# glennhickey/teHmm

Hardware: AMD Instinct MI355X
Metric: genome positions/sec (Viterbi+posterior), 35 states x 10 tracks (higher is better)
Workload: dtype f64

## Files before the change

### include/tehmm_hip.h

```cpp
#ifndef TEHMM_HIP_H
#define TEHMM_HIP_H

#include <stdint.h>

#ifdef __cplusplus
extern "C" {
#endif

#define TEHMM_OK 0
#define TEHMM_ERR_ARG (-1)
#define TEHMM_ERR_HIP (-2)
#define TEHMM_ERR_UNSUPPORTED (-3)

int tehmm_abi_version(void);
const char *tehmm_last_error(void);
int tehmm_device_count(int *count);
int tehmm_set_device(int device);
int tehmm_max_states(void);
int tehmm_max_states_any(void);


int tehmm_emission_u8(int64_t T, int K, int N, int S, const uint8_t *obs, const double *logProbs,
                      double normalize, const double *segRatios, double *outProbs);
int tehmm_emission_u16(int64_t T, int K, int N, int S, const uint16_t *obs, const double *logProbs,
// ... 19 lines not shown
                            const double *posteriors, const double *segRatios);
int tehmm_accumulate_obs_u16(int64_t T, int K, int N, int S, const uint16_t *obs, double *obsStats,
                             const double *posteriors, const double *segRatios);
int tehmm_accumulate_obs_i32(int64_t T, int K, int N, int S, const int32_t *obs, double *obsStats,
                             const double *posteriors, const double *segRatios);

int tehmm_update_counts_u8(int64_t T, int K, int N, int S, const uint8_t *obs, int n_intervals,
                           const int64_t *starts, const int64_t *ends, const int32_t *states,
                           const double *segRatios, double *obsStats);
int tehmm_update_counts_u16(int64_t T, int K, int N, int S, const uint16_t *obs, int n_intervals,
                            const int64_t *starts, const int64_t *ends, const int32_t *states,
                            const double *segRatios, double *obsStats);
int tehmm_update_counts_i32(int64_t T, int K, int N, int S, const int32_t *obs, int n_intervals,
                            const int64_t *starts, const int64_t *ends, const int32_t *states,
                            const double *segRatios, double *obsStats);

typedef struct tehmm_model tehmm_model_t;
typedef struct tehmm_batch tehmm_batch_t;

int tehmm_model_create(int N, int K, int S, const double *log_transmat, const double *log_startprob,
                       const double *logProbs, double normalize, const int32_t *symbolsPerTrack,
                       tehmm_model_t **out);
int tehmm_model_destroy(tehmm_model_t *model);

int tehmm_batch_create(int n_intervals, const int64_t *offsets, int K, const uint8_t *obs,
                       const double *segRatios, int obs_on_device, tehmm_batch_t **out);
int tehmm_batch_create_u16(int n_intervals, const int64_t *offsets, int K, const uint16_t *obs,
                           const double *segRatios, tehmm_batch_t **out);
int tehmm_batch_create_i32(int n_intervals, const int64_t *offsets, int K, const int32_t *obs,
                           const double *segRatios, tehmm_batch_t **out);
int tehmm_batch_destroy(tehmm_batch_t *batch);
int64_t tehmm_batch_total(const tehmm_batch_t *batch);
int tehmm_batch_reset_cache(tehmm_batch_t *batch);

#define TEHMM_EVAL_VITERBI 1
#define TEHMM_EVAL_POSTERIOR 2
#define TEHMM_EVAL_USE_RATIOS 4

int tehmm_eval_batch(tehmm_model_t *model, tehmm_batch_t *batch, int flags,
                     double *viterbi_logprob, double *forward_logprob);

int tehmm_batch_get_paths(tehmm_batch_t *batch, int64_t row0, int64_t row1, int64_t *paths);
int tehmm_batch_get_posteriors(tehmm_batch_t *batch, int64_t row0, int64_t row1, double *post);
int tehmm_host_alloc(size_t bytes, void **out);
int tehmm_host_free(void *ptr);
int tehmm_trim_pools(void);
// ... 44 lines not shown
```

### tehmm_amd/_lib.py

```python
import ctypes
import os

import numpy as np

_HERE = os.path.dirname(os.path.abspath(__file__))
LIB_PATH = os.environ.get("TEHMM_HIP_LIB") or os.path.join(_HERE, "libtehmm_hip.so")

f64p = ctypes.POINTER(ctypes.c_double)
i64p = ctypes.POINTER(ctypes.c_int64)
i32p = ctypes.POINTER(ctypes.c_int32)
u8p = ctypes.POINTER(ctypes.c_uint8)
vp = ctypes.c_void_p
c_i64 = ctypes.c_int64
c_int = ctypes.c_int
c_dbl = ctypes.c_double

SIGNATURES = {
    "tehmm_abi_version": (c_int, []),
    "tehmm_last_error": (ctypes.c_char_p, []),
    "tehmm_device_count": (c_int, [ctypes.POINTER(c_int)]),
    "tehmm_set_device": (c_int, [c_int]),
    "tehmm_max_states": (c_int, []),
    "tehmm_max_states_any": (c_int, []),
    "tehmm_emission_u8": (c_int, [c_i64, c_int, c_int, c_int, vp, f64p, c_dbl, f64p, f64p]),
# ... 21 lines not shown
    "tehmm_model_get_params": (c_int, [vp, f64p, f64p, f64p]),
    "tehmm_segment_table_u8": (c_int, [c_i64, c_int, u8p, c_i64, i64p, u8p, f64p, u8p, f64p]),
    "tehmm_mask_table_u8": (c_int, [c_i64, c_int, u8p, c_int, u8p, u8p, i32p, u8p, i32p, i64p]),
    "tehmm_batch_get_interval_logprobs": (c_int, [vp, f64p]),
    "tehmm_batch_posterior_masksum": (c_int, [vp, f64p, c_i64, c_i64, f64p]),
    "tehmm_bed_coords": (c_int, [c_i64, c_i64, c_i64, i64p, i32p, c_i64, i64p, i64p]),
    "tehmm_write_bed": (c_int, [ctypes.c_char_p, c_int, ctypes.c_char_p, c_i64, i64p, i64p, i64p, c_int,
                                ctypes.POINTER(ctypes.c_char_p), f64p]),
    "tehmm_model_create": (c_int, [c_int, c_int, c_int, f64p, f64p, f64p, c_dbl, i32p,
                                   ctypes.POINTER(vp)]),
    "tehmm_model_destroy": (c_int, [vp]),
    "tehmm_batch_create": (c_int, [c_int, i64p, c_int, vp, vp, c_int, ctypes.POINTER(vp)]),
    "tehmm_batch_create_u16": (c_int, [c_int, i64p, c_int, vp, vp, ctypes.POINTER(vp)]),
    "tehmm_batch_create_i32": (c_int, [c_int, i64p, c_int, vp, vp, ctypes.POINTER(vp)]),
    "tehmm_batch_destroy": (c_int, [vp]),
    "tehmm_batch_total": (c_i64, [vp]),
    "tehmm_batch_reset_cache": (c_int, [vp]),
    "tehmm_eval_batch": (c_int, [vp, vp, c_int, f64p, f64p]),
    "tehmm_batch_get_paths": (c_int, [vp, c_i64, c_i64, i64p]),
    "tehmm_batch_get_posteriors": (c_int, [vp, c_i64, c_i64, f64p]),
    "tehmm_host_alloc": (c_int, [ctypes.c_size_t, ctypes.POINTER(vp)]),
    "tehmm_host_free": (c_int, [vp]),
    "tehmm_trim_pools": (c_int, []),
    "tehmm_batch_device_ptrs": (c_int, [vp, ctypes.POINTER(vp), ctypes.POINTER(vp)]),
    "tehmm_estep_batch": (c_int, [vp, vp, c_int, f64p, f64p, f64p, f64p]),
    "tehmm_batch_last_timing": (c_int, [vp, c_int, ctypes.POINTER(ctypes.c_char_p), f64p]),
    "tehmm_debug_read_stamps": (c_int, [ctypes.POINTER(ctypes.c_uint64), c_int]),
}

EVAL_VITERBI = 1
EVAL_POSTERIOR = 2
EVAL_USE_RATIOS = 4

_lib = None


class TeHmmHipError(RuntimeError):
    code = 0


def load():
    global _lib
    if _lib is None:
        if not os.path.exists(LIB_PATH):
            raise TeHmmHipError(
                "%s not found: build it with `python -m tehmm_amd.build` (hipcc, gfx950). "
# ... 77 lines not shown
```

### tehmm_amd/csrc/tehmm_aux_host.inc

```

int tehmm_segment_table_u8(int64_t T, int K, const uint8_t *data, int64_t n_seg, const int64_t *segOffsets,
                           const uint8_t *is_gaussian, const double *mapback, uint8_t *out, double *means) {
  if (T <= 0 || K <= 0 || K > TEHMM_MAX_TRACKS || n_seg <= 0 || !data || !segOffsets || !is_gaussian || !out || !means)
    return fail(TEHMM_ERR_ARG, "tehmm_segment_table_u8: bad argument");
  bool any_gauss = false;
  for (int k = 0; k < K; ++k) any_gauss = any_gauss || is_gaussian[k] != 0;
  if (any_gauss && !mapback) return fail(TEHMM_ERR_ARG, "tehmm_segment_table_u8: gaussian track without a map-back table");
  for (int64_t i = 0; i < n_seg; ++i)
    if (segOffsets[i] < 0 || segOffsets[i] >= T || (i > 0 && segOffsets[i] <= segOffsets[i - 1]))
      return fail(TEHMM_ERR_ARG, "tehmm_segment_table_u8: segment offsets must be ascending and inside the table");
  DBuf<uint8_t> d_data, d_g, d_out;
  DBuf<int64_t> d_off;
  DBuf<double> d_mb, d_means;
  HIPCHK(d_data.upload(data, (size_t)T * K));
  HIPCHK(d_off.upload(segOffsets, (size_t)n_seg));
  HIPCHK(d_g.upload(is_gaussian, (size_t)K));
  if (mapback) HIPCHK(d_mb.upload(mapback, (size_t)K * 256));
  HIPCHK(d_out.alloc((size_t)n_seg * K));
  HIPCHK(d_means.alloc((size_t)n_seg * K));
  hipLaunchKernelGGL(k_segment_table, dim3(grid_for(n_seg, 4, 16384)), dim3(256), 0, 0, T, K,
                     (const uint8_t *)d_data.p, n_seg, (const int64_t *)d_off.p, (const uint8_t *)d_g.p,
                     (const double *)d_mb.p, d_out.p, d_means.p);
  HIPCHK(hipGetLastError());
  HIPCHK(hipMemcpy(out, d_out.p, (size_t)n_seg * K, hipMemcpyDeviceToHost));
// ... 95 lines not shown
  const int N = m->N, NP = m->NP;
  const MstepTracks tr = mstep_tracks(m);
  if (update_start || update_trans)
    hipLaunchKernelGGL(k_mstep_trans, dim3(1), dim3(128), 0, 0, N, NP, dev_stats, update_start, update_trans,
                       startprob_prior, transmat_prior, m->lt.p, m->pi.p);
  if (update_emission) {
    hipLaunchKernelGGL(k_mstep_emis, dim3(grid_for((int64_t)m->K * N, 64)), dim3(64), 0, 0, tr, N, NP, dev_stats,
                       fudge, m->tab.p);
    if (n_gauss > 0) {
      DBuf<int> d_gt;
      DBuf<double> d_val, d_gp;
      HIPCHK(d_gt.upload(gauss_tracks, (size_t)n_gauss));
      HIPCHK(d_val.upload(gauss_values, (size_t)n_gauss * m->S));
      HIPCHK(d_gp.alloc((size_t)n_gauss * N * 2));
      hipLaunchKernelGGL(k_mstep_gauss, dim3(grid_for((int64_t)n_gauss * N, 64)), dim3(64), 0, 0, tr, n_gauss,
                         (const int *)d_gt.p, (const double *)d_val.p, m->S, N, NP, uniform_mix, m->tab.p, d_gp.p);
      HIPCHK(hipGetLastError());
      if (gauss_params)
        HIPCHK(hipMemcpy(gauss_params, d_gp.p, (size_t)n_gauss * N * 2 * sizeof(double), hipMemcpyDeviceToHost));
      else
        HIPCHK(hipDeviceSynchronize());
    }
    if (int rcp = build_ptab(m)) return rcp;
    if (m->lds_rows > 0) {
      DBuf<int> d_lb;
      HIPCHK(d_lb.upload(m->ldsbase, (size_t)m->K));
      hipLaunchKernelGGL(k_model_ltab, dim3(m->K), dim3(256), 0, 0, tr, (const int *)d_lb.p, NP,
                         (const double *)m->tab.p, m->ltab.p);
      HIPCHK(hipDeviceSynchronize());
    }
  }
  if (update_trans) {
    hipLaunchKernelGGL(k_model_layouts, dim3(grid_for((int64_t)NP * NP, 256)), dim3(256), 0, 0, NP,
                       (const double *)m->lt.p, m->ltT.p, m->A.p, m->AT.p, m->ltG.p, m->AG.p, m->ATG.p, m->ltP.p);
    std::vector<double> hlt((size_t)NP * NP);
    HIPCHK(hipMemcpy(hlt.data(), m->lt.p, hlt.size() * sizeof(double), hipMemcpyDeviceToHost));
    for (int i = 0; i < N; ++i)
      for (int j = 0; j < N; ++j) m->h_lt[(size_t)i * N + j] = hlt[(size_t)i * NP + j];
  }
  HIPCHK(hipGetLastError());
  HIPCHK(hipDeviceSynchronize());
  ++m->version;
  return TEHMM_OK;
}

int tehmm_model_get_params(tehmm_model_t *m, double *log_transmat, double *log_startprob, double *logProbs) {
// ... 24 lines not shown
```

### tehmm_amd/csrc/tehmm_coop.hip.h

```cpp
#pragma once
#include "tehmm_kernels.hip.h"

namespace tehmm {

typedef double d2v __attribute__((ext_vector_type(2)));
typedef __attribute__((address_space(3))) const d2v lds_cd2;
__device__ __forceinline__ lds_cd2 *lds_row(const double *row) {
  unsigned a = (unsigned)(size_t)(__attribute__((address_space(3))) const double *)row;
  asm volatile("v_mov_b32 %0, %1" : "=v"(a) : "v"(a));
  return (lds_cd2 *)(size_t)a;
}

template <int NT>
__device__ __forceinline__ void rep_rows(double v, double (&r)[(NT + 15) / 16]) {
  const unsigned lo = __double2loint(v), hi = __double2hiint(v);
  const auto a = __builtin_amdgcn_permlane32_swap(lo, lo, false, false);
  const auto b = __builtin_amdgcn_permlane32_swap(hi, hi, false, false);
  const auto c = __builtin_amdgcn_permlane16_swap(a[0], a[0], false, false);
  const auto d = __builtin_amdgcn_permlane16_swap(b[0], b[0], false, false);
  r[0] = __hiloint2double((int)d[0], (int)c[0]);
  if constexpr (NT > 16) r[1] = __hiloint2double((int)d[1], (int)c[1]);
  if constexpr (NT > 32) {
    const auto e = __builtin_amdgcn_permlane16_swap(a[1], a[1], false, false);
    const auto f = __builtin_amdgcn_permlane16_swap(b[1], b[1], false, false);
// ... 37 lines not shown

__device__ __forceinline__ double exp_nonpos(double y) {
  const double k = rint(y * 1.4426950408889634);
  double r = fma(k, -6.93147180369123816490e-01, y);
  r = fma(k, -1.90821492927058770002e-10, r);
  double p = 1.6059043836821613e-10;
  p = fma(p, r, 2.08767569878681e-09);
  p = fma(p, r, 2.505210838544172e-08);
  p = fma(p, r, 2.755731922398589e-07);
  p = fma(p, r, 2.7557319223985893e-06);
  p = fma(p, r, 2.48015873015873e-05);
  p = fma(p, r, 1.984126984126984e-04);
  p = fma(p, r, 1.388888888888889e-03);
  p = fma(p, r, 8.333333333333333e-03);
  p = fma(p, r, 4.1666666666666664e-02);
  p = fma(p, r, 1.6666666666666666e-01);
  p = fma(p, r, 0.5);
  p = fma(p, r, 1.0);
  p = fma(p, r, 1.0);
  const double res = ldexp(p, (int)k);
  return y < -1100.0 ? 0.0 : res;
}

template <int NT>
__device__ __forceinline__ void emis_rows(const EmisTab &e, const double *ltab, int64_t gpos,
                                          double (&x)[NT]) {
  const uint32_t *row = e.obs32 + gpos * e.KPW;
#pragma unroll
  for (int j = 0; j < NT; ++j) x[j] = 0.0;
  uint32_t wn = row[0];
  for (int d = 0; d < e.KPW; ++d) {
    const uint32_t w = wn;
    if (d + 1 < e.KPW) wn = row[d + 1];
#pragma unroll
    for (int bb = 0; bb < 4; ++bb) {
      const int k = 4 * d + bb;
      if (k < e.K) {
        const int sym = (int)((w >> (8 * bb)) & 0xffu);
        const bool inr = sym < e.rowcnt[k];
        const int lb = e.ldsbase[k];
        if (lb >= 0) {
          lds_cd2 *tr = (lds_cd2 *)(size_t)((unsigned)(size_t)(
              __attribute__((address_space(3))) const double *)ltab +
              (unsigned)((inr ? lb + sym : e.lds_zero) * NT * 8));
#pragma unroll
          for (int jj = 0; jj < NT / 2; ++jj) {
            const d2v v = tr[jj];
            x[2 * jj] += v.x;
            x[2 * jj + 1] += v.y;
          }
        } else {
          const double2 *tr = (const double2 *)(e.tab + (int64_t)(inr ? e.rowbase[k] + sym : e.zero_row) * NT);
#pragma unroll
          for (int jj = 0; jj < NT / 2; ++jj) {
            const double2 v = tr[jj];
            x[2 * jj] += v.x;
            x[2 * jj + 1] += v.y;
          }
        }
      }
// ... 569 lines not shown
```

### tehmm_amd/csrc/tehmm_hip.hip

```cpp
#include <climits>
#include "tehmm_kernels.hip.h"
#include "tehmm_coop.hip.h"
#include "tehmm_lane.hip.h"
#include "tehmm_lane3.hip.h"
#include "tehmm_place.hip.h"
#include "tehmm_aux.hip.h"
#include "tehmm_fused.hip.h"
#include "tehmm_estep.hip.h"
#include "tehmm_wide_estep.hip.h"
#include "tehmm_wide.hip.h"
#include "tehmm_large.hip.h"

#include <algorithm>
#include <atomic>
#include <cmath>
#include <cstdio>
#include <cstdlib>
#include <cstring>
#include <mutex>
#include <numeric>
#include <string>
#include <thread>
#include <vector>

// ... 199 lines not shown
  if (g > cap) g = cap;
  return (int)g;
}

constexpr int kMaxStates = 128;
#ifndef TEHMM_RATIO_LANE_MAX
#define TEHMM_RATIO_LANE_MAX 64
#endif

int pad_states(int N) {
  static const int sizes[] = {4, 8, 12, 16, 20, 24, 28, 32, 36, 40, 48, 56, 64};
  for (int s : sizes)
    if (N < s) return s;
  return (N + 4) & ~3;
}

template <typename F>
void allow_lds(F *fn, size_t bytes) {
  (void)hipFuncSetAttribute((const void *)fn, hipFuncAttributeMaxDynamicSharedMemorySize, (int)bytes);
}

}

struct tehmm_model {
  int N = 0, NP = 0, K = 0, S = 0, R = 0;
  double normalize = 1.0;
  DBuf<double> lt, ltT, A, AT, pi, tab, ltab;
  DBuf<double> ltG, AG, ATG;
  DBuf<float> ltP;
  DBuf<double> ptab, ptab_lds;
  DBuf<int> d_rowinfo;
  int KSP = 0;
  bool large = false;
  uint64_t uid = 0;
  uint64_t version = 0;
  bool ptab_log = false;
  int rowbase[TEHMM_MAX_TRACKS];
  int rowcnt[TEHMM_MAX_TRACKS];
  int ldsbase[TEHMM_MAX_TRACKS];
  int lds_rows = 0, lds_zero = 0;
  std::vector<double> h_lt;
  DBuf<double> qall[2];
  DBuf<int> qok[2];
  uint64_t q_version[2] = {~(uint64_t)0, ~(uint64_t)0};
};

struct EstepWork {
  DBuf<double> alpha, beta, wrows, fwd_lp;
// ... 301 lines not shown
  HIPCHK(d_e.upload(ends, (size_t)n_iv));
  HIPCHK(d_q.upload(states, (size_t)n_iv));
  if (segRatios) HIPCHK(d_r.upload(segRatios, (size_t)T));
  hipLaunchKernelGGL((k_update_counts<ObsT>), dim3(K, N), dim3(std::min(256, (S + 63) & ~63)), 0, 0, n_iv, d_s.p,
                     d_e.p, d_q.p, K, N, S, d_obs.p, d_st.p, d_r.p);
  HIPCHK(hipGetLastError());
  HIPCHK(hipMemcpy(obsStats, d_st.p, (size_t)K * N * S * sizeof(double), hipMemcpyDeviceToHost));
  return TEHMM_OK;
}

int tehmm_update_counts_u8(int64_t T, int K, int N, int S, const uint8_t *obs, int n_iv, const int64_t *starts,
                           const int64_t *ends, const int32_t *states, const double *segRatios, double *obsStats) {
  return update_counts_impl<uint8_t>(T, K, N, S, obs, n_iv, starts, ends, states, segRatios, obsStats);
}
int tehmm_update_counts_u16(int64_t T, int K, int N, int S, const uint16_t *obs, int n_iv, const int64_t *starts,
                            const int64_t *ends, const int32_t *states, const double *segRatios, double *obsStats) {
  return update_counts_impl<uint16_t>(T, K, N, S, obs, n_iv, starts, ends, states, segRatios, obsStats);
}
int tehmm_update_counts_i32(int64_t T, int K, int N, int S, const int32_t *obs, int n_iv, const int64_t *starts,
                            const int64_t *ends, const int32_t *states, const double *segRatios, double *obsStats) {
  return update_counts_impl<int32_t>(T, K, N, S, obs, n_iv, starts, ends, states, segRatios, obsStats);
}

static int build_ptab(tehmm_model *m) {
  if (m->NP > 64) return TEHMM_OK;
  const int KS = m->NP / 4, KSP = ((KS + 1) + 1) & ~1, ROW_D = 4 * KSP, ROW_L = ROW_D + 2, K = m->K;
  m->KSP = KSP;
  m->ptab_log = m->normalize != 1.0;
  if (!m->ptab.p) {
    HIPCHK(m->ptab.alloc((size_t)(m->R + 1) * ROW_D));
    HIPCHK(m->ptab_lds.alloc((size_t)std::max(1, m->lds_rows) * ROW_L));
    std::vector<int> info((size_t)3 * K);
    for (int k = 0; k < K; ++k) { info[k] = m->rowbase[k]; info[K + k] = m->rowcnt[k]; info[2 * K + k] = m->ldsbase[k]; }
    HIPCHK(m->d_rowinfo.upload(info.data(), info.size()));
  }
  hipLaunchKernelGGL(k_build_ptab, dim3(grid_for(m->R + 1, 64)), dim3(64), 0, 0, m->R + 1, m->N, m->NP, KSP,
                     (const double *)m->tab.p, m->ptab_log ? 1 : 0, m->ptab.p);
  if (m->lds_rows > 0)
    hipLaunchKernelGGL(k_pack_ptab_lds, dim3(K + 1), dim3(256), 0, 0, K, (const int *)m->d_rowinfo.p,
                       (const int *)m->d_rowinfo.p + K, (const int *)m->d_rowinfo.p + 2 * K, m->lds_zero, m->R, ROW_D,
                       ROW_L, (const double *)m->ptab.p, m->ptab_lds.p);
  HIPCHK(hipGetLastError());
  HIPCHK(hipDeviceSynchronize());
  return TEHMM_OK;
}

// ... 146 lines not shown
  for (int f = 0; f < NP; ++f)
    for (int o = 0; o < NP; ++o) hltP[((size_t)(o >> 1) * NP + f) * 2 + (o & 1)] = (float)hlt[(size_t)f * NP + o];
  for (int o = 0; o < N; ++o) hltP[(size_t)NP * NP + o] = (float)hlt[(size_t)o * NP + o];
  hltP[(size_t)NP * NP + NP] = (float)hlt[0];
  if (e == hipSuccess) e = m->ltG.upload(hltG.data(), hltG.size());
  if (e == hipSuccess) e = m->ltP.upload(hltP.data(), hltP.size());
  if (e == hipSuccess) e = m->AG.upload(hAG.data(), hAG.size());
  if (e == hipSuccess) e = m->ATG.upload(hATG.data(), hATG.size());
  if (e == hipSuccess) e = m->ltT.upload(hltT.data(), hltT.size());
  if (e == hipSuccess) e = m->ltab.upload(hltab.data(), hltab.size());
  if (e == hipSuccess) e = m->A.upload(hA.data(), hA.size());
  if (e == hipSuccess) e = m->AT.upload(hAT.data(), hAT.size());
  if (e == hipSuccess) e = m->pi.upload(hpi.data(), hpi.size());
  htab.resize(htab.size() + 64, 0.0);
  if (e == hipSuccess) e = m->tab.upload(htab.data(), htab.size());
  if (e != hipSuccess) {
    delete m;
    return fail(TEHMM_ERR_HIP, std::string("tehmm_model_create: ") + hipGetErrorString(e));
  }
  if (int rc = build_ptab(m)) {
    delete m;
    return rc;
  }
  *out = m;
  return TEHMM_OK;
}

int tehmm_model_destroy(tehmm_model_t *model) {
  delete model;
  return TEHMM_OK;
}

namespace {
struct StreamSet {
  int dev;
  hipStream_t sV, sP, sB;
  hipEvent_t evX[2], ev[16];
};
std::mutex g_sset_mu;
std::vector<StreamSet> g_sset;
bool stream_set_take(tehmm_batch *b) {
  const int dev = dev_current();
  std::lock_guard<std::mutex> lk(g_sset_mu);
  for (size_t i = 0; i < g_sset.size(); ++i)
    if (g_sset[i].dev == dev) {
      const StreamSet ss = g_sset[i];
// ... 204 lines not shown
  em.obs32 = (const uint32_t *)b->obs.p;
  em.tab = m->tab.p;
  em.ratios = emis_ratios ? b->ratios.p : nullptr;
  em.normalize = m->normalize;
  em.K = m->K;
  em.KPW = b->KP / 4;
  em.NP = m->NP;
  std::memcpy(em.rowbase, m->rowbase, sizeof(em.rowbase));
  std::memcpy(em.rowcnt, m->rowcnt, sizeof(em.rowcnt));
  std::memcpy(em.ldsbase, m->ldsbase, sizeof(em.ldsbase));
  em.lds_rows = m->lds_rows;
  em.ltab_src = m->ltab.p;
  em.zero_row = m->R;
  em.lds_zero = m->lds_zero;
}

static EmisTab without_lds_tables(const EmisTab &em) {
  EmisTab e = em;
  e.lds_rows = 0;
  for (int k = 0; k < TEHMM_MAX_TRACKS; ++k) e.ldsbase[k] = -1;
  return e;
}

static int ensure_workspace(tehmm_batch *b, const tehmm_model *m, int flags) {
  if (b->N != m->N) {
    b->paths.release();
    b->post.release();
    b->tb.release();
    b->G.release();
    b->beta.release();
    b->N = m->N;
    b->NP = m->NP;
    b->TBW = m->NP;
  }
  if ((flags & TEHMM_EVAL_VITERBI) && !b->paths.p) {
    HIPCHK(b->paths.alloc((size_t)b->total + 1));
    HIPCHK(b->tb.alloc((size_t)(b->total_pad + 1) * b->TBW));
    HIPCHK(b->G.alloc((size_t)(b->n_chunks + 1) * b->NP));
    HIPCHK(b->bstate.alloc((size_t)b->n_chunks + 1));
    HIPCHK(b->last_state.alloc((size_t)b->n + 1));
    HIPCHK(b->vit_lp.alloc((size_t)b->n + 1));
  }
  if ((flags & TEHMM_EVAL_POSTERIOR) && !b->post.p) {
    HIPCHK(b->post.alloc((size_t)b->total * m->N + 1));
    HIPCHK(b->fwd_lp.alloc((size_t)b->n + 1));
    HIPCHK(b->first_good.alloc((size_t)b->n + 1));
// ... 94 lines not shown
                     m->lt.p, m->pi.p, (const double *)nullptr, b->post.p, b->beta.p, b->fwd_lp.p,
                     b->dead.p, (double *)nullptr, (int *)nullptr);
}

static int spec_chunk_size() {
  const char *s = std::getenv("TEHMM_SPEC_CHUNK");
  int cs = s ? std::atoi(s) : 512;
  if (cs <= 0) return 0;
  return std::max(64, (cs + 63) & ~63);
}

struct EvalKnobs {
  int spec_chunk;
  int lane_sub;
  int lane_warmup;
  bool lane_probe;
  bool lane_vit;
  bool lane_p0;
  bool fused;
  bool device_place;
  bool soft_ties;
  int emis_split;
  int defer;
};

static EvalKnobs read_eval_knobs() {
  auto num = [](const char *name, int unset) {
    const char *s = std::getenv(name);
    return s ? std::atoi(s) : unset;
  };
  EvalKnobs k;
  k.spec_chunk = spec_chunk_size();
  k.lane_sub = std::getenv("TEHMM_LANE_SUB") ? std::max(0, num("TEHMM_LANE_SUB", 0)) : -1;
  k.lane_warmup = std::getenv("TEHMM_LANE_WARMUP") ? std::max(1, num("TEHMM_LANE_WARMUP", 1)) : -1;
  k.lane_probe = num("TEHMM_LANE_PROBE", 1) != 0;
  k.lane_vit = num("TEHMM_LANE_VIT", 1) != 0;
  k.lane_p0 = num("TEHMM_LANE_P0", 1) != 0;
  k.fused = num("TEHMM_FUSED", 1) != 0;
  k.device_place = num("TEHMM_DEVICE_PLACE", 1) != 0;
  k.soft_ties = num("TEHMM_SOFT_TIES", 1) != 0;
  k.emis_split = std::getenv("TEHMM_EMIS_SPLIT") ? (num("TEHMM_EMIS_SPLIT", 0) != 0 ? 1 : 0) : -1;
  k.defer = num("TEHMM_DEFER", -1);
  return k;
}

static int spec_prepare(tehmm_batch *b, const tehmm_model *m, int CS) {
  SpecWork &sw = b->sw;
  if (sw.CS == CS && sw.N == m->N && sw.rows.p) return TEHMM_OK;
  sw.CS = CS;
  sw.N = m->N;
  sw.h_iv.clear();
  sw.h_t0.clear();
  sw.h_first.assign((size_t)b->n + 1, 0);
  for (int i = 0; i < b->n; ++i) {
    sw.h_first[i] = (int64_t)sw.h_iv.size();
    for (int64_t t0 = 0; t0 < b->h_len[i]; t0 += CS) {
      sw.h_iv.push_back(i);
      sw.h_t0.push_back(t0);
    }
  }
  sw.h_first[b->n] = (int64_t)sw.h_iv.size();
  sw.n_chunks = (int)sw.h_iv.size();
  const size_t nc = (size_t)std::max(1, sw.n_chunks);
  HIPCHK(sw.iv.upload(sw.h_iv.data(), sw.h_iv.size()));
  HIPCHK(sw.t0.upload(sw.h_t0.data(), sw.h_t0.size()));
// ... 355 lines not shown
  *n_work_max = 2 * lw.n_groups + TEHMM_PLACE_NE;
  return TEHMM_OK;
}

template <int NT>
static void launch_vit_stitch(tehmm_batch *b, const tehmm_model *m, const IntervalTab &iv, const VitChunks &vc,
                              hipStream_t st) {
  LaneWork &lw = b->lw;
  hipLaunchKernelGGL((k_vit_stitch<NT>), dim3((vc.n + 3) / 4), dim3(256), 0, st, iv, lane_geom(lw), vc,
                     lane_vit_items(lw), m->N, lw.soft_ties);
  hipLaunchKernelGGL((k_vit_links<NT>), dim3((vc.n + 3) / 4), dim3(256), 0, st, iv, lane_geom(lw), vc,
                     lane_vit_items(lw), m->N);
  hipLaunchKernelGGL(k_vit_runs, dim3(std::max(1, b->n)), dim3(64), 0, st, vc, b->n);
}

static LaneGeom lane_geom(const LaneWork &lw) {
  LaneGeom lg;
  lg.item_iv = lw.item_iv.p; lg.item_t0 = lw.item_t0.p; lg.ifirst = lw.ifirst.p;
  lg.n_items = lw.n_items; lg.n_groups = lw.n_groups; lg.L = lw.L;
  return lg;
}

template <int NT>
static void launch_emis_lane(tehmm_batch *b, const tehmm_model *m, const IntervalTab &iv, const EmisTab &em,
                             bool want_log, bool want_lin, bool want_f32, hipStream_t st) {
  LaneWork &lw = b->lw;
  const size_t lds = (size_t)em.lds_rows * NT * sizeof(double);
  allow_lds(k_emis_lane<NT>, lds);
  hipLaunchKernelGGL((k_emis_lane<NT>), dim3((lw.n_groups + 3) / 4), dim3(256), lds, st, iv, em, lane_geom(lw),
                     m->N, want_log ? lw.B.p : (double *)nullptr, want_lin ? lw.BH.p : (double *)nullptr, lw.MS.p,
                     want_f32 ? lw.B32.p : (float *)nullptr);
}

template <int NT>
static void launch_emis_gain_lane(tehmm_batch *b, const tehmm_model *m, const IntervalTab &iv, const EmisTab &em,
                                  int CS, int Wu, bool ratio, int emis_split, hipStream_t st) {
  LaneWork &lw = b->lw;
  if constexpr (NT >= 12) {
    const bool split = emis_split >= 0 ? emis_split != 0 : lw.n_groups < 2048;
    if (split) {
      constexpr int NW = TEHMM_P2_NW, NU = 2;
      const size_t lds3 = Emis3Geom<NT, NW, NU>::lds_bytes(em.lds_rows);
      const dim3 grid3((lw.n_groups + NU - 1) / NU);
      if constexpr (NT <= TEHMM_RATIO_LANE_MAX) if (ratio) {
        allow_lds(k_emis_gain_lane3<NT, NW, NU, true>, lds3);
        hipLaunchKernelGGL((k_emis_gain_lane3<NT, NW, NU, true>), grid3, dim3(64 * NW * NU), lds3, st, iv, em, lane_geom(lw),
                           m->N, CS, Wu, (const float *)m->ltP.p, lw.B.p, lw.vgain.p, (const double *)b->ratios.p);
        return;
      }
      allow_lds(k_emis_gain_lane3<NT, NW, NU, false>, lds3);
      hipLaunchKernelGGL((k_emis_gain_lane3<NT, NW, NU, false>), grid3, dim3(64 * NW * NU), lds3, st, iv, em, lane_geom(lw),
                         m->N, CS, Wu, (const float *)m->ltP.p, lw.B.p, lw.vgain.p, (const double *)nullptr);
      return;
    }
  }
  const size_t lds = (size_t)em.lds_rows * NT * sizeof(double);
  if constexpr (NT <= TEHMM_RATIO_LANE_MAX) if (ratio) {
    allow_lds(k_emis_gain_lane<NT, true>, lds);
    hipLaunchKernelGGL((k_emis_gain_lane<NT, true>), dim3((lw.n_groups + 3) / 4), dim3(256), lds, st, iv, em,
                       lane_geom(lw), m->N, CS, Wu, (const float *)m->ltP.p, lw.B.p, lw.vgain.p,
// ... 959 lines not shown
  HIPCHK(lw.wk_items.ensure((ng + TEHMM_PLACE_NE) * 64));
  HIPCHK(lw.gclass.ensure(ng));
  HIPCHK(lw.place.ensure(1));
  HIPCHK(hipMemsetAsync(lw.place.p, 0, sizeof(PlaceCounts), st));
  HIPCHK(hipMemsetAsync(lw.wk_items.p, 0xff, (ng + TEHMM_PLACE_NE) * 64 * sizeof(int), st));
  HIPCHK(hipMemsetAsync(sw.ok.p, 0, (size_t)std::max(1, sw.n_chunks) * sizeof(int), st));
  HIPCHK(hipMemsetAsync(sw.stats.p, 0, 2 * sizeof(int), st));
  HIPCHK(hipMemsetAsync(lw.vbad.p, 0, ng * 64 * sizeof(int), st));
  HIPCHK(hipMemsetAsync(lw.vntie.p, 0, ng * 64 * sizeof(int), st));
  return vit_lane_upload_args(b, c.vc, st);
}

static int eval_emis_p0(EvalCtx &c) {
  tehmm_batch *b = c.b;
  const tehmm_model *m = c.m;
  const EvalPlan &p = c.p;
  LaneWork &lw = b->lw;
  SpecWork &sw = b->sw;
  std::vector<double> &gain = lw.hs_gain;
  hipStream_t st = b->sV;
  if (p.vlane || p.glane) {
    if (p.emis_gain) {
      nt_dispatch(m->NP, [&](auto nt) {
        launch_emis_gain_lane<nt>(b, m, c.iv, c.em, p.CS, p.WuV, p.ratio, c.kn.emis_split, st);
      });
    } else {
      nt_dispatch(m->NP, [&](auto nt) {
        launch_emis_lane<nt>(b, m, c.iv, c.em, p.vlane, p.flane && !p.fused_fb, p.glane, st);
      });
    }
    (void)hipEventRecord(b->ev[eV + 4], st);
    if (p.flane) {
      if (!p.fused_fb) {
        (void)hipEventRecord(b->evX[0], st);
        (void)hipStreamWaitEvent(b->sP, b->evX[0], 0);
      }
      (void)hipEventRecord(b->ev[eP + 4], b->sP);
    }
  }
  if (p.vspec) {
    if (p.glane) {
      if (!p.emis_gain) nt_dispatch(m->NP, [&](auto nt) { launch_gain_lane<nt>(b, m, c.iv, p.CS, p.WuV, st); });
      if (!p.dev_place) {
        gain.resize((size_t)std::max(1, lw.n_groups) * 64);
        HIPCHK(hipMemcpyAsync(gain.data(), lw.vgain.p, gain.size() * sizeof(double), hipMemcpyDeviceToHost, st));
      }
    } else {
      nt_dispatch(m->NP, [&](auto nt) { launch_vit_spec<nt>(b, m, c.iv, c.emg, c.vc, false, st); });
      gain.resize((size_t)std::max(1, sw.n_chunks));
      HIPCHK(hipMemcpyAsync(gain.data(), sw.gain.p, gain.size() * sizeof(double), hipMemcpyDeviceToHost, st));
    }
  }
  return TEHMM_OK;
}

static void eval_emission(EvalCtx &c) {
  const EvalPlan &p = c.p;
  if (!(p.flane && !p.fused_fb && !p.vlane && !p.glane)) return;
  tehmm_batch *b = c.b;
  hipStream_t st = b->sP;
  nt_dispatch(c.m->NP, [&](auto nt) { launch_emis_lane<nt>(b, c.m, c.iv, c.em, false, true, false, st); });
  (void)hipEventRecord(b->ev[eP + 4], st);
}

static int eval_posterior(EvalCtx &c, int half) {
  tehmm_batch *b = c.b;
  const tehmm_model *m = c.m;
  const EvalPlan &p = c.p;
  const IntervalTab &iv = c.iv;
  LaneWork &lw = b->lw;
  SpecWork &sw = b->sw;
  hipStream_t st = b->sP;
  int rc = TEHMM_OK;
  if (half != 2) (void)hipEventRecord(b->ev[10], st);
  else (void)hipEventRecord(b->ev[11], st);
  if (p.flane) {
    FbChunks fc{};
    fc.iv = sw.iv.p; fc.t0 = sw.t0.p; fc.first = sw.first.p; fc.n = sw.n_chunks; fc.CS = p.CS;
    fc.scale = sw.scale.p; fc.wstart = sw.wstart.p;
    fc.link_f = lw.link_f.p; fc.glog_f = lw.glog_f.p; fc.link_b = lw.link_b.p; fc.runend_f = lw.runend_f.p;
    fc.pre_f = lw.cpre_f.p; fc.runstart_b = lw.runstart_b.p;
    if (half != 2) {
      (void)hipMemsetAsync(b->dead.p, 0, (size_t)(b->n + 1) * sizeof(int), st);
      (void)hipMemsetAsync(sw.stats.p + 2, 0, 4 * sizeof(int), st);
// ... 1576 lines not shown
```

### tehmm_amd/csrc/tehmm_kernels.hip.h

```cpp
#pragma once
#include <hip/hip_runtime.h>
#include <stdint.h>

#define TEHMM_WAVE 64
#ifndef TEHMM_PRIO_HI
#define TEHMM_PRIO_HI 3
#define TEHMM_PRIO_LO 2
#endif
#define TEHMM_MAX_TRACKS 128
#define TEHMM_PB 16
#define TEHMM_TB_CHUNK 256

namespace tehmm {

#ifdef TEHMM_STAMPS
__device__ unsigned long long g_stamps[2 * 4096 * 16];
__device__ __forceinline__ unsigned long long stamp_now() {
  unsigned long long t;
  asm volatile("s_memtime %0\n\ts_waitcnt lgkmcnt(0)" : "=s"(t)::"memory");
  return t;
}
#define ST_DECL unsigned long long st_a = 0, st_b = 0, st_c = 0, st_t0 = 0, st_t1 = 0
#define ST_BEGIN st_t0 = stamp_now()
#define ST_ADD(acc) do { st_t1 = stamp_now(); acc += st_t1 - st_t0; st_t0 = st_t1; } while (0)
// ... 4 lines not shown
      g_stamps[(blockIdx.x * 4 + (w_)) * 4 + 1] = st_b;                                     \
      g_stamps[(blockIdx.x * 4 + (w_)) * 4 + 2] = st_c;                                     \
    }                                                                                       \
  } while (0)
#else
#define ST_DECL
#define ST_BEGIN
#define ST_ADD(acc)
#define ST_FLUSH(w_)
#endif

struct EmisTab {
  const uint32_t *obs32;
  const double *tab;
  const double *ratios;
  double normalize;
  int K, KPW, NP;
  int rowbase[TEHMM_MAX_TRACKS];
  int rowcnt[TEHMM_MAX_TRACKS];
  int ldsbase[TEHMM_MAX_TRACKS];
  int lds_rows;
  const double *ltab_src;
  int zero_row, lds_zero;
};

struct IntervalTab {
  const int *order;
  const int64_t *pos0;
  const int64_t *len;
  const int64_t *out0;
  int n;
};

__device__ __forceinline__ double wave_max_f64(double v) {
#pragma unroll
  for (int o = 32; o > 0; o >>= 1) v = fmax(v, __shfl_xor(v, o));
  return v;
}
__device__ __forceinline__ double wave_sum_f64(double v) {
#pragma unroll
  for (int o = 32; o > 0; o >>= 1) v += __shfl_xor(v, o);
  return v;
}
__device__ __forceinline__ int wave_max_i32(int v) {
#pragma unroll
  for (int o = 32; o > 0; o >>= 1) v = max(v, __shfl_xor(v, o));
  return v;
// ... 1345 lines not shown
```

### tehmm_amd/csrc/tehmm_lane3.hip.h

```cpp
#pragma once
#include "tehmm_lane.hip.h"

namespace tehmm {

#ifndef TEHMM_P2_NW
#define TEHMM_P2_NW 3
#endif
#ifndef TEHMM_L3_EXP
#define TEHMM_L3_EXP 0
#endif
typedef double lane3_d2 __attribute__((ext_vector_type(2)));
typedef __attribute__((address_space(1))) double lane3_gf64;
typedef __attribute__((address_space(1))) int lane3_gi32;
#define LANE3_G(p) ((lane3_gf64 *)(p))
#define LANE3_GI(p) ((lane3_gi32 *)(p))
template <typename T>
__device__ __forceinline__ T lane3_gload(T const *p) {
  return *(const __attribute__((address_space(1))) T *)p;
}

#ifdef TEHMM_STAMPS
#define L3ST(i) do { const unsigned long long n_ = stamp_now(); l3st[i] += n_ - l3tt; l3tt = n_; } while (0)
#else
#define L3ST(i) do { } while (0)
// ... 389 lines not shown
        for (int j = 0; j < NT; ++j) dst[po + ((int64_t)j << 6)] = W[j] * 0.015625 + base;
        LANE3_GI(lane3_gload(&vi->ntie))[item] = nt;
        LANE3_G(lane3_gload(&vi->piecemin))[item * (TEHMM_LANE_MAXTI + 1) + min(nt, TEHMM_LANE_MAXTI)] = pm;
      }
      if (anybad) LANE3_GI(lane3_gload(&vi->bad))[item] = 1;
    }
  }
}

}

namespace tehmm {

template <int NT, int NW, int NU>
struct Emis3Geom {
  using L3 = Lane3Geom<NT, NW>;
  static constexpr size_t UNIT_BYTES = (size_t)2 * (NT / 2) * 64 * sizeof(float) * 2 + (size_t)2 * NW * 64 * sizeof(double);
  static size_t lds_bytes(int lds_rows) { return (size_t)lds_rows * NT * sizeof(double) + NU * UNIT_BYTES; }
};

template <int NT, int NS>
__device__ __forceinline__ void emis_rows_slice(const EmisTab &e, const double *ltab, int64_t gpos, int j0, double (&x)[NS]) {
  const uint32_t *row = e.obs32 + gpos * e.KPW;
#pragma unroll
  for (int j = 0; j < NS; ++j) x[j] = 0.0;
  uint32_t wn = row[0];
  for (int d = 0; d < e.KPW; ++d) {
    const uint32_t w = wn;
    if (d + 1 < e.KPW) wn = row[d + 1];
#pragma unroll
    for (int bb = 0; bb < 4; ++bb) {
      const int k = 4 * d + bb;
      if (k < e.K) {
        const int sym = (int)((w >> (8 * bb)) & 0xffu);
        const bool inr = sym < e.rowcnt[k];
        const int lb = e.ldsbase[k];
        if (lb >= 0) {
          lds_cd2 *tr = (lds_cd2 *)(size_t)((unsigned)(size_t)(__attribute__((address_space(3))) const double *)ltab +
                                            (unsigned)(((inr ? lb + sym : e.lds_zero) * NT + j0) * 8));
#pragma unroll
          for (int jj = 0; jj < NS / 2; ++jj) {
            const d2v v = tr[jj];
            x[2 * jj] += v.x;
            x[2 * jj + 1] += v.y;
          }
        } else {
          const double2 *tr = (const double2 *)(e.tab + (int64_t)(inr ? e.rowbase[k] + sym : e.zero_row) * NT + j0);
#pragma unroll
          for (int jj = 0; jj < NS / 2; ++jj) {
            const double2 v = tr[jj];
            x[2 * jj] += v.x;
            x[2 * jj + 1] += v.y;
          }
        }
      }
    }
// ... 126 lines not shown
```

Baseline: 1.522 billion.

## Precompute joint emission table for leading tracks to cut per-position LDS lookups

Builds a combined table on the host that holds the summed emission rows for every symbol combination of the first 2-4 tracks, sized to fit a 32 KB LDS budget. The emission kernels then do one LDS row fetch for those tracks instead of one fetch and add per track. This cuts LDS traffic and add instructions in the per-position emission loop. In exchange it spends extra LDS, builds the table on the host at model creation and after each M-step, and computes the prefix sum in a different addition order, which can change the low bits of the f64 results.

```diff
diff --git a/include/tehmm_hip.h b/include/tehmm_hip.h
--- a/include/tehmm_hip.h
+++ b/include/tehmm_hip.h
@@ -65,6 +65,7 @@
                        const double *logProbs, double normalize, const int32_t *symbolsPerTrack,
                        tehmm_model_t **out);
 int tehmm_model_destroy(tehmm_model_t *model);
+int tehmm_joint_prefix_table(int p, const int32_t *rowcnt, int NP, const double *rows, double *out);
 
 int tehmm_batch_create(int n_intervals, const int64_t *offsets, int K, const uint8_t *obs,
                        const double *segRatios, int obs_on_device, tehmm_batch_t **out);
diff --git a/tehmm_amd/_lib.py b/tehmm_amd/_lib.py
--- a/tehmm_amd/_lib.py
+++ b/tehmm_amd/_lib.py
@@ -67,6 +67,7 @@
     "tehmm_host_alloc": (c_int, [ctypes.c_size_t, ctypes.POINTER(vp)]),
     "tehmm_host_free": (c_int, [vp]),
     "tehmm_trim_pools": (c_int, []),
+    "tehmm_joint_prefix_table": (c_int, [c_int, i32p, c_int, f64p, f64p]),
     "tehmm_batch_device_ptrs": (c_int, [vp, ctypes.POINTER(vp), ctypes.POINTER(vp)]),
     "tehmm_estep_batch": (c_int, [vp, vp, c_int, f64p, f64p, f64p, f64p]),
     "tehmm_batch_last_timing": (c_int, [vp, c_int, ctypes.POINTER(ctypes.c_char_p), f64p]),
diff --git a/tehmm_amd/csrc/tehmm_aux_host.inc b/tehmm_amd/csrc/tehmm_aux_host.inc
--- a/tehmm_amd/csrc/tehmm_aux_host.inc
+++ b/tehmm_amd/csrc/tehmm_aux_host.inc
@@ -141,6 +141,11 @@
         HIPCHK(hipDeviceSynchronize());
     }
     if (int rcp = build_ptab(m)) return rcp;
+    if (m->K >= 2) {
+      std::vector<double> htab((size_t)(m->R + 1) * NP);
+      HIPCHK(hipMemcpy(htab.data(), m->tab.p, htab.size() * sizeof(double), hipMemcpyDeviceToHost));
+      if (int rcl = build_lane_tabs(m, htab.data())) return rcl;
+    }
     if (m->lds_rows > 0) {
       DBuf<int> d_lb;
       HIPCHK(d_lb.upload(m->ldsbase, (size_t)m->K));
diff --git a/tehmm_amd/csrc/tehmm_coop.hip.h b/tehmm_amd/csrc/tehmm_coop.hip.h
--- a/tehmm_amd/csrc/tehmm_coop.hip.h
+++ b/tehmm_amd/csrc/tehmm_coop.hip.h
@@ -83,20 +83,39 @@
   return y < -1100.0 ? 0.0 : res;
 }
 
+__device__ __forceinline__ int joint_prefix_index(const EmisTab &e, uint32_t w0) {
+  int idx = e.jbase;
+#pragma unroll
+  for (int k = 0; k < 4; ++k)
+    if (k < e.jp) idx += min((int)((w0 >> (8 * k)) & 0xffu), e.rowcnt[k]) * e.jstride[k];
+  return idx;
+}
+
 template <int NT>
 __device__ __forceinline__ void emis_rows(const EmisTab &e, const double *ltab, int64_t gpos,
                                           double (&x)[NT]) {
   const uint32_t *row = e.obs32 + gpos * e.KPW;
-#pragma unroll
-  for (int j = 0; j < NT; ++j) x[j] = 0.0;
   uint32_t wn = row[0];
+  if (e.jp > 0) {
+    lds_cd2 *tr = (lds_cd2 *)(size_t)((unsigned)(size_t)(
+        __attribute__((address_space(3))) const double *)ltab + (unsigned)(joint_prefix_index(e, wn) * NT * 8));
+#pragma unroll
+    for (int jj = 0; jj < NT / 2; ++jj) {
+      const d2v v = tr[jj];
+      x[2 * jj] = v.x;
+      x[2 * jj + 1] = v.y;
+    }
+  } else {
+#pragma unroll
+    for (int j = 0; j < NT; ++j) x[j] = 0.0;
+  }
   for (int d = 0; d < e.KPW; ++d) {
     const uint32_t w = wn;
     if (d + 1 < e.KPW) wn = row[d + 1];
 #pragma unroll
     for (int bb = 0; bb < 4; ++bb) {
       const int k = 4 * d + bb;
-      if (k < e.K) {
+      if (k < e.K && k >= e.jp) {
         const int sym = (int)((w >> (8 * bb)) & 0xffu);
         const bool inr = sym < e.rowcnt[k];
         const int lb = e.ldsbase[k];
diff --git a/tehmm_amd/csrc/tehmm_hip.hip b/tehmm_amd/csrc/tehmm_hip.hip
--- a/tehmm_amd/csrc/tehmm_hip.hip
+++ b/tehmm_amd/csrc/tehmm_hip.hip
@@ -245,8 +245,17 @@
 
 }
 
+struct LaneTabs {
+  int jp = 0, n_joint = 0, lds_rows = 0, lds_zero = 0;
+  int jstride[4] = {0, 0, 0, 0};
+  int ldsbase[TEHMM_MAX_TRACKS];
+  DBuf<double> ltab;
+};
+static constexpr size_t kLaneTabBudget = 32 * 1024;
+
 struct tehmm_model {
   int N = 0, NP = 0, K = 0, S = 0, R = 0;
+  LaneTabs lane_tabs;
   double normalize = 1.0;
   DBuf<double> lt, ltT, A, AT, pi, tab, ltab;
   DBuf<double> ltG, AG, ATG;
@@ -594,6 +603,82 @@
   return update_counts_impl<int32_t>(T, K, N, S, obs, n_iv, starts, ends, states, segRatios, obsStats);
 }
 
+static void joint_prefix_build(int p, const int *cnt, int NP, const double *rows, double *out) {
+  const int64_t n = joint_prefix_rows(p, cnt);
+  for (int64_t r = 0; r < n; ++r)
+    for (int j = 0; j < NP; ++j) {
+      double acc = 0.0;
+      int64_t rem = r;
+      const double *trk = rows;
+      for (int k = 0; k < p; ++k) {
+        const int digit = (int)(rem % (cnt[k] + 1));
+        rem /= cnt[k] + 1;
+        acc = acc + (digit < cnt[k] ? trk[(size_t)digit * NP + j] : 0.0);
+        trk += (size_t)cnt[k] * NP;
+      }
+      out[(size_t)r * NP + j] = acc;
+    }
+}
+
+static int plan_lane_tabs(const tehmm_model *m, size_t budget, LaneTabs &lt) {
+  const size_t budget_rows = budget / ((size_t)m->NP * sizeof(double));
+  lt.jp = 0;
+  for (int p = std::min(4, m->K); p >= 2; --p) {
+    size_t rows = 1;
+    for (int k = p; k < m->K; ++k)
+      if (m->ldsbase[k] >= 0) rows += (size_t)m->rowcnt[k];
+    size_t nj = 1;
+    for (int k = 0; k < p && nj <= budget_rows; ++k) nj *= (size_t)m->rowcnt[k] + 1;
+    if (nj + rows > budget_rows) continue;
+    lt.jp = p;
+    lt.n_joint = (int)nj;
+    int stride = 1, used = (int)nj;
+    for (int k = 0; k < m->K; ++k) {
+      lt.ldsbase[k] = -1;
+      if (k < p) {
+        lt.jstride[k] = stride;
+        stride *= m->rowcnt[k] + 1;
+      } else if (m->ldsbase[k] >= 0) {
+        lt.ldsbase[k] = used;
+        used += m->rowcnt[k];
+      }
+    }
+    lt.lds_zero = used;
+    lt.lds_rows = used + 1;
+    break;
+  }
+  return lt.jp;
+}
+
+static int build_lane_tabs(tehmm_model *m, const double *htab) {
+  const int NP = m->NP;
+  LaneTabs &lt = m->lane_tabs;
+  if (!plan_lane_tabs(m, kLaneTabBudget, lt)) return TEHMM_OK;
+  std::vector<double> h((size_t)lt.lds_rows * NP, 0.0);
+  joint_prefix_build(lt.jp, m->rowcnt, NP, htab + (size_t)m->rowbase[0] * NP, h.data());
+  for (int k = lt.jp; k < m->K; ++k)
+    if (lt.ldsbase[k] >= 0)
+      std::memcpy(&h[(size_t)lt.ldsbase[k] * NP], htab + (size_t)m->rowbase[k] * NP,
+                  (size_t)m->rowcnt[k] * NP * sizeof(double));
+  if (lt.ltab.p && lt.ltab.n == h.size())
+    HIPCHK(hipMemcpy(lt.ltab.p, h.data(), h.size() * sizeof(double), hipMemcpyHostToDevice));
+  else
+    HIPCHK(lt.ltab.upload(h.data(), h.size()));
+  return TEHMM_OK;
+}
+
+int tehmm_joint_prefix_table(int p, const int32_t *rowcnt, int NP, const double *rows, double *out) {
+  if (p < 1 || p > 4 || NP < 1 || !rowcnt || !rows || !out)
+    return fail(TEHMM_ERR_ARG, "tehmm_joint_prefix_table: bad argument");
+  int cnt[4];
+  for (int k = 0; k < p; ++k) {
+    if (rowcnt[k] < 1 || rowcnt[k] > 257) return fail(TEHMM_ERR_ARG, "tehmm_joint_prefix_table: bad row count");
+    cnt[k] = rowcnt[k];
+  }
+  joint_prefix_build(p, cnt, NP, rows, out);
+  return TEHMM_OK;
+}
+
 static int build_ptab(tehmm_model *m) {
   if (m->NP > 64) return TEHMM_OK;
   const int KS = m->NP / 4, KSP = ((KS + 1) + 1) & ~1, ROW_D = 4 * KSP, ROW_L = ROW_D + 2, K = m->K;
@@ -786,6 +871,10 @@
     delete m;
     return rc;
   }
+  if (int rc = build_lane_tabs(m, htab.data())) {
+    delete m;
+    return rc;
+  }
   *out = m;
   return TEHMM_OK;
 }
@@ -1036,6 +1125,20 @@
   return e;
 }
 
+static EmisTab with_lane_tabs(const EmisTab &em, const tehmm_model *m, bool joint) {
+  const LaneTabs &lt = m->lane_tabs;
+  if (!joint || lt.jp == 0 || em.lds_rows == 0) return em;
+  EmisTab e = em;
+  std::memcpy(e.ldsbase, lt.ldsbase, sizeof(e.ldsbase));
+  e.lds_rows = lt.lds_rows;
+  e.lds_zero = lt.lds_zero;
+  e.ltab_src = lt.ltab.p;
+  e.jp = lt.jp;
+  e.jbase = 0;
+  std::memcpy(e.jstride, lt.jstride, sizeof(e.jstride));
+  return e;
+}
+
 static int ensure_workspace(tehmm_batch *b, const tehmm_model *m, int flags) {
   if (b->N != m->N) {
     b->paths.release();
@@ -1176,6 +1279,7 @@
   bool soft_ties;
   int emis_split;
   int defer;
+  bool joint_tabs;
 };
 
 static EvalKnobs read_eval_knobs() {
@@ -1195,6 +1299,7 @@
   k.soft_ties = num("TEHMM_SOFT_TIES", 1) != 0;
   k.emis_split = std::getenv("TEHMM_EMIS_SPLIT") ? (num("TEHMM_EMIS_SPLIT", 0) != 0 ? 1 : 0) : -1;
   k.defer = num("TEHMM_DEFER", -1);
+  k.joint_tabs = num("TEHMM_JOINT_TABS", 1) != 0;
   return k;
 }
 
@@ -1596,9 +1701,10 @@
 }
 
 template <int NT>
-static void launch_emis_lane(tehmm_batch *b, const tehmm_model *m, const IntervalTab &iv, const EmisTab &em,
-                             bool want_log, bool want_lin, bool want_f32, hipStream_t st) {
+static void launch_emis_lane(tehmm_batch *b, const tehmm_model *m, const IntervalTab &iv, const EmisTab &em_in,
+                             bool want_log, bool want_lin, bool want_f32, bool joint, hipStream_t st) {
   LaneWork &lw = b->lw;
+  const EmisTab em = with_lane_tabs(em_in, m, joint);
   const size_t lds = (size_t)em.lds_rows * NT * sizeof(double);
   allow_lds(k_emis_lane<NT>, lds);
   hipLaunchKernelGGL((k_emis_lane<NT>), dim3((lw.n_groups + 3) / 4), dim3(256), lds, st, iv, em, lane_geom(lw),
@@ -1607,9 +1713,10 @@
 }
 
 template <int NT>
-static void launch_emis_gain_lane(tehmm_batch *b, const tehmm_model *m, const IntervalTab &iv, const EmisTab &em,
-                                  int CS, int Wu, bool ratio, int emis_split, hipStream_t st) {
+static void launch_emis_gain_lane(tehmm_batch *b, const tehmm_model *m, const IntervalTab &iv, const EmisTab &em_in,
+                                  int CS, int Wu, bool ratio, int emis_split, bool joint, hipStream_t st) {
   LaneWork &lw = b->lw;
+  const EmisTab em = with_lane_tabs(em_in, m, joint);
   if constexpr (NT >= 12) {
     const bool split = emis_split >= 0 ? emis_split != 0 : lw.n_groups < 2048;
     if (split) {
@@ -2615,11 +2722,11 @@
   if (p.vlane || p.glane) {
     if (p.emis_gain) {
       nt_dispatch(m->NP, [&](auto nt) {
-        launch_emis_gain_lane<nt>(b, m, c.iv, c.em, p.CS, p.WuV, p.ratio, c.kn.emis_split, st);
+        launch_emis_gain_lane<nt>(b, m, c.iv, c.em, p.CS, p.WuV, p.ratio, c.kn.emis_split, c.kn.joint_tabs, st);
       });
     } else {
       nt_dispatch(m->NP, [&](auto nt) {
-        launch_emis_lane<nt>(b, m, c.iv, c.em, p.vlane, p.flane && !p.fused_fb, p.glane, st);
+        launch_emis_lane<nt>(b, m, c.iv, c.em, p.vlane, p.flane && !p.fused_fb, p.glane, c.kn.joint_tabs, st);
       });
     }
     (void)hipEventRecord(b->ev[eV + 4], st);
@@ -2652,7 +2759,7 @@
   if (!(p.flane && !p.fused_fb && !p.vlane && !p.glane)) return;
   tehmm_batch *b = c.b;
   hipStream_t st = b->sP;
-  nt_dispatch(c.m->NP, [&](auto nt) { launch_emis_lane<nt>(b, c.m, c.iv, c.em, false, true, false, st); });
+  nt_dispatch(c.m->NP, [&](auto nt) { launch_emis_lane<nt>(b, c.m, c.iv, c.em, false, true, false, c.kn.joint_tabs, st); });
   (void)hipEventRecord(b->ev[eP + 4], st);
 }
 
diff --git a/tehmm_amd/csrc/tehmm_kernels.hip.h b/tehmm_amd/csrc/tehmm_kernels.hip.h
--- a/tehmm_amd/csrc/tehmm_kernels.hip.h
+++ b/tehmm_amd/csrc/tehmm_kernels.hip.h
@@ -50,7 +50,15 @@
   int lds_rows;
   const double *ltab_src;
   int zero_row, lds_zero;
+  int jp = 0, jbase = 0;
+  int jstride[4] = {0, 0, 0, 0};
 };
+
+__host__ __device__ inline int64_t joint_prefix_rows(int p, const int *cnt) {
+  int64_t n = 1;
+  for (int k = 0; k < p; ++k) n *= cnt[k] + 1;
+  return n;
+}
 
 struct IntervalTab {
   const int *order;
diff --git a/tehmm_amd/csrc/tehmm_lane3.hip.h b/tehmm_amd/csrc/tehmm_lane3.hip.h
--- a/tehmm_amd/csrc/tehmm_lane3.hip.h
+++ b/tehmm_amd/csrc/tehmm_lane3.hip.h
@@ -435,16 +435,27 @@
 template <int NT, int NS>
 __device__ __forceinline__ void emis_rows_slice(const EmisTab &e, const double *ltab, int64_t gpos, int j0, double (&x)[NS]) {
   const uint32_t *row = e.obs32 + gpos * e.KPW;
-#pragma unroll
-  for (int j = 0; j < NS; ++j) x[j] = 0.0;
   uint32_t wn = row[0];
+  if (e.jp > 0) {
+    lds_cd2 *tr = (lds_cd2 *)(size_t)((unsigned)(size_t)(__attribute__((address_space(3))) const double *)ltab +
+                                      (unsigned)((joint_prefix_index(e, wn) * NT + j0) * 8));
+#pragma unroll
+    for (int jj = 0; jj < NS / 2; ++jj) {
+      const d2v v = tr[jj];
+      x[2 * jj] = v.x;
+      x[2 * jj + 1] = v.y;
+    }
+  } else {
+#pragma unroll
+    for (int j = 0; j < NS; ++j) x[j] = 0.0;
+  }
   for (int d = 0; d < e.KPW; ++d) {
     const uint32_t w = wn;
     if (d + 1 < e.KPW) wn = row[d + 1];
 #pragma unroll
     for (int bb = 0; bb < 4; ++bb) {
       const int k = 4 * d + bb;
-      if (k < e.K) {
+      if (k < e.K && k >= e.jp) {
         const int sym = (int)((w >> (8 * bb)) & 0xffu);
         const bool inr = sym < e.rowcnt[k];
         const int lb = e.ldsbase[k];
```

Result: no change. 1.530 billion, median of 6 (+0.5%).
